# nickgreenquist/cu2rec

Measured on AMD Instinct MI355X. Metric: ratings/sec (SGD updates/sec), higher is better.
Workload: dtype f32

## Files before the change

cu2rec_amd/csrc/blocksolve.hip:

```cpp
#include <hip/hip_runtime.h>
#include <hip/hip_ext.h>

#include <algorithm>
#include <atomic>
#include <cmath>
#include <cstdlib>
#include <limits>
#include <mutex>
#include <string>
#include <utility>
#include <vector>

#include "blocksolve.hpp"
#include "blocksolve_device.hpp"
#include "blocksolve_gram.hpp"
#include "blocksolve_lookahead.hpp"
#include "blocksolve_solve.hpp"
#include "blocksolve_update.hpp"
#include "hip_check.hpp"

namespace cu2rec {

namespace {

using namespace bs_dev;

__global__ void bs_tables_kernel(SgdHyper h, float *__restrict__ t) {
    const int k = threadIdx.x;
    if (k > 2 * kB) return;
    const double a = 1.0 - static_cast<double>(h.lr) * static_cast<double>(h.q_reg);
    const double c = 1.0 - static_cast<double>(h.lr) * static_cast<double>(h.ib_reg);
    double ak = 1.0, ck = 1.0;
    for (int i = 0; i < k; ++i) {
        ak *= a;
        ck *= c;
    }
    t[kTabAdel + k] = static_cast<float>(1.0 - ak);
    t[kTabCdel + k] = static_cast<float>(1.0 - ck);
    t[kTabApow + k] = static_cast<float>(ak);
    t[kTabCpow + k] = static_cast<float>(ck);
}

__device__ __forceinline__ int lower_bound_key(const uint32_t *__restrict__ keys, int n, uint32_t target) {
    int lo = 0, hi = n;
    while (lo < hi) {
        const int mid = (lo + hi) >> 1;
        if (keys[mid] < target) lo = mid + 1; else hi = mid;
    }
    return lo;
}

__global__ __launch_bounds__(256) void bs_plan_kernel(const uint32_t *__restrict__ keys, int n_active, int n_hot,
                                                      int item_bits, int max_blocks, const int *__restrict__ item_of_rank,
                                                      int *__restrict__ chain_begin, BsChainDesc *__restrict__ chains,
                                                      BsBlockDesc *__restrict__ blocks, int *__restrict__ walk_begin, size_t stride) {
    __shared__ int s_part[256];
    const int b = blockIdx.x, tid = threadIdx.x;
    const uint32_t *kb = keys + static_cast<size_t>(b) * stride;
    int *cb = chain_begin + static_cast<size_t>(b) * (n_hot + 1);
    BsChainDesc *cd = chains + static_cast<size_t>(b) * max(n_hot, 1);
    BsBlockDesc *bd = blocks + static_cast<size_t>(b) * max_blocks;
    for (int r = tid; r <= n_hot; r += 256) cb[r] = lower_bound_key(kb, n_active, static_cast<uint32_t>(r));
    __syncthreads();
    if (tid == 0) walk_begin[b] = cb[n_hot];
    const int per = (n_hot + 255) / 256;
    const int r0 = min(tid * per, n_hot), r1 = min(r0 + per, n_hot);
    int mine = 0;
    for (int r = r0; r < r1; ++r) mine += (cb[r + 1] - cb[r] + kB - 1) / kB;
    s_part[tid] = mine;
    __syncthreads();
    __shared__ int s_total;
    if (tid == 0) {
        int run = 0;
        for (int t = 0; t < 256; ++t) {
            const int v = s_part[t];
            s_part[t] = run;
            run += v;
        }
        s_total = run;
    }
    __syncthreads();
    int off = s_part[tid];
    for (int r = r0; r < r1; ++r) {
        const int begin = cb[r], len = cb[r + 1] - begin;
        cd[r] = BsChainDesc{begin, len, off, item_of_rank[r]};
        const int nb = (len + kB - 1) / kB;
        for (int m = 0; m < nb; ++m) bd[off + m] = BsBlockDesc{begin + kB * m, min(kB, len - kB * m), r, m};
        off += nb;
    }
    for (int g = s_total + tid; g < max_blocks; g += 256) bd[g] = BsBlockDesc{0, 0, 0, 0};
}

__global__ __launch_bounds__(256, 4) void bs_gram_kernel(SgdArgs a, BsIteration it) {
    extern __shared__ float4 bs_smem[];
    const int g = static_cast<int>(blockIdx.x) - it.la_grid;
    __builtin_amdgcn_s_setprio(2);
    struct Through {
        unsigned long long *count;
        __device__ ~Through() {
            if (count && threadIdx.x == 0)
                __hip_atomic_fetch_add(count + 16 * (blockIdx.x & 31), 1ull, __ATOMIC_RELAXED, __HIP_MEMORY_SCOPE_AGENT);
        }
    } through_count{it.gram_done};
    if (g < 0) {
        const BsChainDesc last = it.chains[it.la_ranks - 1];
        const int la_end = min(last.blk0 + (last.len + kB - 1) / kB, it.la_cap);
        for (int gb = g + it.la_grid; gb < la_end; gb += it.la_grid) gram_cross_block(a, it, gb, bs_smem);
        return;
    }
    gram_block(a, it, g, bs_smem);
}

template <int SW>
__global__ __launch_bounds__(512) void bs_solve_kernel(SgdArgs a, BsIteration it) {
    extern __shared__ float4 bs_smem[];
    if (it.gram_done && threadIdx.x == 0)
        __hip_atomic_fetch_add(it.solve_started, 1ull, __ATOMIC_RELAXED, __HIP_MEMORY_SCOPE_AGENT);
    const int chain = blockIdx.x;
    const BsChainDesc cd = it.chains[chain];
    if constexpr (SW <= 8) {
        if (chain_is_lookahead(it, chain, cd)) {
            chain_lookahead<(4 * SW < kLaMaxSlots ? 4 * SW : kLaMaxSlots)>(a, it, bs_smem, cd);
            return;
        }
    }
    solve_chain<SW>(a, it, bs_smem, cd);
}

__global__ __launch_bounds__(64 * kUpdMaxWaves) void bs_update_kernel(SgdArgs a, BsIteration it) {
    const int g = blockIdx.x;
    __builtin_amdgcn_s_setprio(2);
    if (g == it.launch_blocks) {
        if (threadIdx.x == 0) await_iteration_end(it);
        return;
    }
    for (int blk = g; blk < it.max_blocks; blk += it.launch_blocks) {
        if (it.blocks[blk].n_valid == 0) break;
        update_block(a, it, blk);
    }
}

template <int SW>
void launch_solve_sw(const SgdArgs &a, const BsIteration &it, hipStream_t stream) {
    size_t lds = solve_lds_bytes(a.nslots, SW);
    if (it.la_ranks > 0) lds = std::max(lds, la_lds_bytes(a.nslots));
    ensure_max_dynamic_lds(reinterpret_cast<const void *>(bs_solve_kernel<SW>));
    hipLaunchKernelGGL((bs_solve_kernel<SW>), dim3(it.n_hot), dim3(512), lds, stream, a, it);
    const hipError_t err = hipGetLastError();
    if (err != hipSuccess)
        fail(CU2REC_EHIP, std::string("bs_solve_kernel launch failed: ") + hipGetErrorString(err) + " (SW " + std::to_string(SW) +
                              ", chains " + std::to_string(it.n_hot) + ", LDS " + std::to_string(lds) + " bytes)");
}

}

namespace {
__global__ void bs_probe_wait_kernel(const unsigned *word, unsigned *result, unsigned long long ticks) {
    if (threadIdx.x != 0) return;
    const unsigned long long t0 = wall_clock64();
    unsigned seen = 0;
    for (;;) {
        if (ld_agent(word) != 0u) {
            seen = 1;
            break;
        }
        __builtin_amdgcn_s_sleep(8);
        if (wall_clock64() - t0 > ticks) break;
    }
    __hip_atomic_store(result, seen ? 1u : 2u, __ATOMIC_RELAXED, __HIP_MEMORY_SCOPE_AGENT);
}

__global__ void bs_probe_signal_kernel(unsigned *word) {
    if (threadIdx.x == 0) __hip_atomic_store(word, 1u, __ATOMIC_RELAXED, __HIP_MEMORY_SCOPE_AGENT);
}

bool probe_streams(hipStream_t waiter, hipStream_t signaller, unsigned *scratch) {
    CU2REC_HIP(hipMemsetAsync(scratch, 0, 64 * sizeof(unsigned), waiter));
    CU2REC_HIP(hipStreamSynchronize(waiter));
    CU2REC_HIP(hipStreamSynchronize(signaller));
    hipLaunchKernelGGL(bs_probe_wait_kernel, dim3(1), dim3(64), 0, waiter, scratch, scratch + 32, 1000000ull);
    hipLaunchKernelGGL(bs_probe_signal_kernel, dim3(1), dim3(64), 0, signaller, scratch);
    CU2REC_HIP(hipGetLastError());
    CU2REC_HIP(hipStreamSynchronize(waiter));
    CU2REC_HIP(hipStreamSynchronize(signaller));
    unsigned result = 0;
    CU2REC_HIP(hipMemcpy(&result, scratch + 32, sizeof(unsigned), hipMemcpyDeviceToHost));
    return result == 1u;
}

int topology(DeviceRuntime &r, hipStream_t stream, hipStream_t side) {
    if (r.topology >= 0) return r.topology;
    if (const char *env = std::getenv("CU2REC_BS_GATE")) {
        r.topology = std::atoi(env) != 0 ? DeviceRuntime::kTopologyDevice : DeviceRuntime::kTopologyEvents;
        r.topology_forced = true;
        r.topology_why = std::string("CU2REC_BS_GATE=") + env;
        return r.topology;
    }
    if (const char *pmc = std::getenv("ROCPROF_COUNTER_COLLECTION"))
        if (*pmc && std::string(pmc) != "0" && std::string(pmc) != "False" && std::string(pmc) != "false") {
            r.topology = DeviceRuntime::kTopologyEvents;
            r.topology_why = "a rocprofv3 counter pass (ROCPROF_COUNTER_COLLECTION) serialises kernels across streams";
            return r.topology;
        }
    const bool forward = probe_streams(stream, side, r.probe);
    const bool backward = forward && probe_streams(side, stream, r.probe);
    if (forward && backward) {
        r.topology = DeviceRuntime::kTopologyDevice;
        r.topology_why = "two-stream handshake probe passed in both directions";
    } else {
        r.topology = DeviceRuntime::kTopologyEvents;
        r.topology_why = std::string("two-stream handshake probe: a wait kernel on the ") + (forward ? "side" : "main") +
                         " stream was not reached by the other stream's signal kernel within 10 ms (the streams do not run side by side here)";
    }
    return r.topology;
}

unsigned long long wait_ticks() {
    static const unsigned long long ticks = [] {
        double sec = 2.0;
        if (const char *env = std::getenv("CU2REC_BS_WAIT_S")) sec = std::max(0.001, std::atof(env));
        return static_cast<unsigned long long>(sec * 1e8);
    }();
    return ticks;
}

#ifdef CU2REC_TEST_HOOKS
int dbg() {
    static const int bits = std::getenv("CU2REC_BS_DBG") ? std::atoi(std::getenv("CU2REC_BS_DBG")) : 0;
    return bits;
}
#else
constexpr int dbg() { return 0; }
#endif

__global__ void bs_gate_kernel(const unsigned long long *count, unsigned long long target, const unsigned long long *started,
                               unsigned long long started_target, unsigned long long wait_ticks) {
    const int lane = threadIdx.x;
    const unsigned long long t0 = wall_clock64();
    unsigned polls = 0;
    for (;;) {
        unsigned long long v = lane < 32 ? ld_agent(count + 16 * lane) : 0ull;
#pragma unroll
        for (int off = 16; off > 0; off >>= 1) v += __shfl_xor(v, off);
        const unsigned long long sum = __shfl(v, 0);
        const unsigned long long st = ld_agent(started);
        if (sum >= target && st >= started_target) break;
        __builtin_amdgcn_s_sleep(16);
        if ((++polls & 63u) == 0 && wall_clock64() - t0 > wait_ticks) break;
    }
}

__global__ void bs_signal_kernel(unsigned long long *word, unsigned long long value) {
    if (threadIdx.x == 0) __hip_atomic_store(word, value, __ATOMIC_RELAXED, __HIP_MEMORY_SCOPE_AGENT);
}

void launch_gram(const SgdArgs &a, const BsIteration &it, hipStream_t stream, hipEvent_t stop) {
    const size_t gram_lds = gram_lds_bytes(a.nslots, it.la_ranks > 0);
    ensure_max_dynamic_lds(reinterpret_cast<const void *>(bs_gram_kernel));
    const int grid = it.max_blocks + (it.la_ranks > 0 ? it.la_grid : 0);
    if (stop) hipExtLaunchKernelGGL(bs_gram_kernel, dim3(grid), dim3(256), static_cast<uint32_t>(gram_lds), stream, nullptr, stop, 0, a, it);
    else hipLaunchKernelGGL(bs_gram_kernel, dim3(grid), dim3(256), gram_lds, stream, a, it);
    CU2REC_HIP(hipGetLastError());
}

void launch_solve(const SgdArgs &a, const BsIteration &it, hipStream_t stream) {
    const int sw = (a.nslots + 3) / 4;
    if (sw <= 1) launch_solve_sw<1>(a, it, stream);
    else if (sw <= 2) launch_solve_sw<2>(a, it, stream);
    else if (sw <= 4) launch_solve_sw<4>(a, it, stream);
    else if (sw <= 7) launch_solve_sw<7>(a, it, stream);
    else if (sw <= 8) launch_solve_sw<8>(a, it, stream);
    else if (sw <= 12) launch_solve_sw<12>(a, it, stream);
    else if (sw <= 16) launch_solve_sw<16>(a, it, stream);
    else fail(CU2REC_EUNSUPPORTED, "block-solve mode is compiled for n_factors <= 252");
}

void launch_update(const SgdArgs &a, const BsIteration &it, hipStream_t stream) {
    const int nwaves = (4 * a.nslots + 63) / 64;
    hipLaunchKernelGGL(bs_update_kernel, dim3(it.launch_blocks + (it.side_seq ? 1 : 0)), dim3(64 * nwaves), 0, stream, a, it);
    CU2REC_HIP(hipGetLastError());
}

std::atomic<int> g_lookahead{-1};
std::atomic<float> g_min_rate{-2.f};
constexpr float kDefaultRate = 240.f;

float min_rate_state() {
    float cur = g_min_rate.load();
    if (cur == -2.f) {
        float init = -1.f;
        if (const char *env = std::getenv("CU2REC_BLOCKSOLVE_RATE")) init = std::max(0.01f, static_cast<float>(std::atof(env)));
        g_min_rate.compare_exchange_strong(cur, init);
        cur = g_min_rate.load();
    }
    return cur;
}
}

int blocksolve_lookahead_blocks(int blocks) {
    int prev = g_lookahead.load();
    if (prev < 0) {
        const char *env = std::getenv("CU2REC_BLOCKSOLVE_LOOKAHEAD");
        const int init = env ? std::max(0, std::atoi(env)) : 24;
        g_lookahead.compare_exchange_strong(prev, init);
        prev = g_lookahead.load();
    }
    if (blocks >= 0) g_lookahead.store(blocks);
    return prev;
}

float blocksolve_min_rate(float rate) {
    const float prev = min_rate_state();
    if (rate > 0.f) g_min_rate.store(rate);
    else if (rate < 0.f) g_min_rate.store(-1.f);
    return prev > 0.f ? prev : -1.f;
}

int blocksolve_hot_items(const std::vector<double> &rate, int n_active, int rank_limit) {
    const float state = min_rate_state();
    float min_rate = state > 0.f ? state : kDefaultRate;
    const int n_cols = static_cast<int>(rate.size());
    if (state <= 0.f) {
        min_rate = std::max(30.f, min_rate * static_cast<float>(n_active) / 131072.f);
        if (n_cols > 0 && n_active <= 131072 / 4 && rate[0] < 350.0) min_rate = rate[0] >= 150.0 ? 60.f : std::numeric_limits<float>::infinity();
    }
    int n = 0;
    while (n < n_cols && rate[n] >= min_rate) ++n;
    return std::min(n, rank_limit);
}

BlockSolve::BlockSolve(int n_hot_, const std::vector<double> &rate, double hot_rate, int n_active_, int item_bits_, int max_batch_,
                       const int *item_of_rank_)
    : n_hot(n_hot_), n_active(n_active_), item_bits(item_bits_), max_batch(max_batch_), item_of_rank(item_of_rank_) {
    max_blocks = n_active / kBsLinks + n_hot + 1;
    const double bound = (hot_rate + 8.0 * std::sqrt(hot_rate) + 64.0) / kBsLinks + n_hot + 1;
    launch_blocks = std::max(1, bound >= static_cast<double>(max_blocks) ? max_blocks : static_cast<int>(bound));
    if (dbg() & 512) launch_blocks = std::min(3, max_blocks);
    const int la_min = blocksolve_lookahead_blocks(-1);
    double la_blocks = 0.0;
    while (la_min > 0 && la_ranks < n_hot && rate[la_ranks] >= static_cast<double>(la_min) * kBsLinks) {
        la_blocks += std::ceil(rate[la_ranks] / kBsLinks) + 1.0;
        ++la_ranks;
    }
    if (la_ranks > 0) la_cap = std::min(max_blocks, static_cast<int>(la_blocks * 1.25) + 4 * la_ranks + 8);
    for (int slot = 0; slot < 2; ++slot) {
        chain_begin[slot].allocate(static_cast<size_t>(max_batch) * (n_hot + 1));
        walk_begin[slot].allocate(max_batch);
        chains[slot].allocate(static_cast<size_t>(max_batch) * n_hot);
        blocks[slot].allocate(static_cast<size_t>(max_batch) * max_blocks);
    }
    tables.allocate(kBsTableFloats);
    Mbuf.allocate(static_cast<size_t>(max_blocks) * kBsRecFloats);
    ebuf.allocate(static_cast<size_t>(max_blocks) * kBsLinks);
    solve_started.allocate(16);
    solve_started.zero();
    gram_done.allocate(32 * 16);
    gram_done.zero();
    side_seq.allocate(16);
    side_seq.zero();
    if (la_cap > 0) Nbuf.allocate(static_cast<size_t>(la_cap) * kBsCrossFloats);
}

BlockSolve::~BlockSolve() {
    if (upd) (void)hipStreamDestroy(upd);
    for (hipEvent_t e : {ev_call, ev_upd, ev_gram})
        if (e) (void)hipEventDestroy(e);
}

void BlockSolve::plan(int slot, const uint32_t *sk, int nb, size_t stride, hipStream_t sched) {
    hipLaunchKernelGGL(bs_plan_kernel, dim3(nb), dim3(256), 0, sched, sk, n_active, n_hot, item_bits, max_blocks, item_of_rank,
                       chain_begin[slot].ptr, chains[slot].ptr, blocks[slot].ptr, walk_begin[slot].ptr, stride);
}

void BlockSolve::begin(const SgdArgs &a, hipStream_t stream) {
    if (a.nslots < 1 || a.nslots > kBsMaxSlots) fail(CU2REC_EUNSUPPORTED, "block-solve mode is compiled for n_factors <= 252");
    const bool same = tables_valid && tables_for.lr == a.h.lr && tables_for.q_reg == a.h.q_reg && tables_for.ib_reg == a.h.ib_reg;
    if (!same) {
        hipLaunchKernelGGL(bs_tables_kernel, dim3(1), dim3(192), 0, stream, a.h, tables.ptr);
        tables_for = a.h;
        tables_valid = true;
    }
    if (qstart_ld != a.ldq) {
        CU2REC_HIP(hipStreamSynchronize(stream));
        qstart.allocate(static_cast<size_t>(max_blocks) * a.ldq);
        qstart_ld = a.ldq;
    }
    if (!upd) {
        CU2REC_HIP(hipStreamCreateWithFlags(&upd, hipStreamNonBlocking));
        for (hipEvent_t *e : {&ev_call, &ev_upd, &ev_gram}) CU2REC_HIP(hipEventCreateWithFlags(e, hipEventDisableTiming));
    }
    unsigned *status = nullptr;
    {
        std::lock_guard<std::mutex> lock(device_runtime_mutex());
        DeviceRuntime &r = device_runtime();
        device_join = topology(r, stream, upd) == DeviceRuntime::kTopologyDevice;
        status = r.status + DeviceRuntime::kBlocksolveWord;
        host_status = r.host_status + 1;
    }
    CU2REC_HIP(hipEventRecord(ev_call, stream));
    CU2REC_HIP(hipStreamWaitEvent(upd, ev_call, 0));
    const bool la_on = la_ranks > 0 && la_supported(a.nslots);
    it = BsIteration{};
    it.n_active = n_active;
    it.n_hot = n_hot;
    it.item_mask = (1u << item_bits) - 1u;
    it.item_of_rank = item_of_rank;
    it.tables = tables.ptr;
    it.log2a = static_cast<float>(std::log2(1.0 - static_cast<double>(a.h.lr) * static_cast<double>(a.h.q_reg)));
    it.log2c = static_cast<float>(std::log2(1.0 - static_cast<double>(a.h.lr) * static_cast<double>(a.h.ib_reg)));
    it.Mbuf = Mbuf.ptr;
    it.ebuf = ebuf.ptr;
    it.qstart = qstart.ptr;
    it.max_blocks = max_blocks;
    it.launch_blocks = launch_blocks;
    it.la_ranks = la_on ? la_ranks : 0;
    it.la_cap = la_cap;
    it.la_grid = la_on ? la_cap : 0;
    it.Nbuf = Nbuf.ptr;
    it.status = status;
    it.solve_started = solve_started.ptr;
    it.wait_ticks = wait_ticks();
    if (device_join) {
        it.gram_done = gram_done.ptr;
        it.side_seq = side_seq.ptr;
    }
    upd_pending = false;
}

void BlockSolve::iteration(const SgdArgs &a, int slot, int b, const uint32_t *keys, const uint64_t *vals, bool last, hipStream_t stream,
                           const SideChains &side) {
    it.keys = keys;
    it.vals = vals;
    it.chains = chains[slot].ptr + static_cast<size_t>(b) * n_hot;
    it.blocks = blocks[slot].ptr + static_cast<size_t>(b) * max_blocks;
    it.walk_begin = walk_begin[slot].ptr + b;
    it.side_target = device_join ? side_seq_host + 1 : 0;
    if (upd_pending) CU2REC_HIP(hipStreamWaitEvent(stream, ev_upd, 0));
    launch_gram(a, it, stream, device_join ? nullptr : ev_gram);
    if (device_join) gram_done_target += static_cast<unsigned long long>(max_blocks + it.la_grid);
    else CU2REC_HIP(hipStreamWaitEvent(upd, ev_gram, 0));
    launch_solve(a, it, stream);
    if (device_join) {
        started_total += static_cast<unsigned long long>(n_hot);
        hipLaunchKernelGGL(bs_gate_kernel, dim3(1), dim3(64), 0, upd, gram_done.ptr, gram_done_target + ((dbg() & 32) ? (1ull << 40) : 0ull),
                           solve_started.ptr, started_total, it.wait_ticks);
        CU2REC_HIP(hipGetLastError());
    }
    side(upd, !device_join || last ? ev_upd : nullptr);
    if (device_join) {
        ++side_seq_host;
        if (!(dbg() & 16)) {
            hipLaunchKernelGGL(bs_signal_kernel, dim3(1), dim3(64), 0, upd, side_seq.ptr, side_seq_host);
            CU2REC_HIP(hipGetLastError());
        }
    }
    launch_update(a, it, stream);
    upd_pending = !device_join;
}

void BlockSolve::join(hipStream_t stream) {
    CU2REC_HIP(hipStreamWaitEvent(stream, ev_upd, 0));
    upd_pending = false;
}

void BlockSolve::end(hipStream_t stream) {
    CU2REC_HIP(hipMemcpyAsync(host_status, it.status, sizeof(unsigned), hipMemcpyDeviceToHost, stream));
}

}
```

cu2rec_amd/csrc/blocksolve.hpp:

```cpp
#pragma once

#include <functional>
#include <vector>

#include <hip/hip_runtime.h>

#include <cstddef>
#include <cstdint>

#include "hip_check.hpp"
#include "kernels.hpp"

namespace cu2rec {

constexpr int kBsLinks = 64;
constexpr int kBsTableStride = 2 * kBsLinks + 1;
constexpr int kBsTableFloats = 4 * kBsTableStride;
constexpr int kBsFactorFloats = 3 * 32 * 32;
constexpr int kBsRecFloats = kBsFactorFloats + kBsLinks;
constexpr int kBsCrossFloats = kBsLinks * kBsLinks;
constexpr int kBsMaxSlots = 63;

struct BsBlockDesc {
    int pos0;
    int n_valid;
    int chain;
    int m;
};

struct BsChainDesc {
    int begin, len;
    int blk0;
    int item;
};

struct BsIteration {
    const uint32_t *keys;
    const uint64_t *vals;
    int n_active;
    int n_hot;
    uint32_t item_mask;
    const BsChainDesc *chains;
    const BsBlockDesc *blocks;
    const int *walk_begin;
    const int *item_of_rank;
    const float *tables;
    float log2a, log2c;
    float *Mbuf;
    float *ebuf;
    float *qstart;
    int max_blocks;
    int launch_blocks;
    int la_ranks;
    int la_cap;
    int la_grid;
    float *Nbuf;
    unsigned *status;
    unsigned long long *solve_started;
    const unsigned long long *side_seq;
    unsigned long long side_target;
    unsigned long long *gram_done;
    unsigned long long wait_ticks;
};

float blocksolve_min_rate(float rate);
int blocksolve_lookahead_blocks(int blocks);
int blocksolve_hot_items(const std::vector<double> &rate, int n_active, int rank_limit);

class BlockSolve {
public:
    BlockSolve(int n_hot, const std::vector<double> &rate, double hot_rate, int n_active, int item_bits, int max_batch,
               const int *item_of_rank);
    ~BlockSolve();
    BlockSolve(const BlockSolve &) = delete;
    BlockSolve &operator=(const BlockSolve &) = delete;
    void plan(int slot, const uint32_t *sk, int nb, size_t stride, hipStream_t sched);
    void begin(const SgdArgs &a, hipStream_t stream);
    using SideChains = std::function<void(hipStream_t side, hipEvent_t stop)>;
    void iteration(const SgdArgs &a, int slot, int b, const uint32_t *keys, const uint64_t *vals, bool last, hipStream_t stream,
                   const SideChains &side);
    void join(hipStream_t stream);
    void end(hipStream_t stream);

    const int n_hot;

private:
    int n_active, item_bits, max_batch;
    const int *item_of_rank;
    int max_blocks;
    int launch_blocks;
    int la_ranks = 0;
    int la_cap = 0;
    DeviceBuffer<int> chain_begin[2], walk_begin[2];
    DeviceBuffer<BsChainDesc> chains[2];
    DeviceBuffer<BsBlockDesc> blocks[2];
    DeviceBuffer<float> tables, Mbuf, ebuf, qstart, Nbuf;
    int qstart_ld = 0;
    SgdHyper tables_for{};
    bool tables_valid = false;
    DeviceBuffer<unsigned long long> solve_started, gram_done, side_seq;
    unsigned long long gram_done_target = 0, started_total = 0, side_seq_host = 0;
    hipStream_t upd = nullptr;
    hipEvent_t ev_call = nullptr, ev_upd = nullptr, ev_gram = nullptr;
    BsIteration it{};
    bool device_join = false;
    bool upd_pending = false;
    unsigned *host_status = nullptr;
};

}
```

cu2rec_amd/csrc/ordered.hip:

```cpp
#include <hip/hip_runtime.h>
#include <hip/hip_ext.h>

#include <cstring>
#include <rocprim/rocprim.hpp>

#include <algorithm>
#include <atomic>
#include <cmath>
#include <cstdio>
#include <cstdlib>
#include <limits>
#include <map>
#include <mutex>
#include <numeric>
#include <string>
#include <vector>

#include "hip_check.hpp"
#include "item_rates.hpp"
#include "kernels.hpp"
#include "ordered.hpp"
#include "sampler.hpp"
#include "sgd_device.hpp"

namespace cu2rec {

namespace {

using namespace dev;

constexpr unsigned kSegBlock = 1024;
constexpr unsigned kSegItems = 8;
using SegSortConfig = rocprim::segmented_radix_sort_config<8, rocprim::kernel_config<kSegBlock, kSegItems>,
                                                           rocprim::WarpSortConfig<8, 4, 256, 64, 16, 8, 256>, true>;

constexpr int kHotChains = 256;

__device__ __forceinline__ int lower_bound_key(const uint32_t *__restrict__ keys, int n, uint32_t target) {
    int lo = 0, hi = n;
    while (lo < hi) {
        const int mid = (lo + hi) >> 1;
        if (keys[mid] < target) lo = mid + 1; else hi = mid;
    }
    return lo;
}

constexpr int kRowRounds = 8;
constexpr int kTileStride = 65;

__global__ __launch_bounds__(256) void schedule_keys_tile_kernel(const int *__restrict__ indptr, const int *__restrict__ indices,
                                                                 const float *__restrict__ data, const int *__restrict__ item_rank,
                                                                 int n_rows, int n_batch, int item_bits, uint32_t sentinel, uint64_t seed,
                                                                 uint64_t iter0, int user_offset, uint32_t *__restrict__ keys,
                                                                 uint64_t *__restrict__ vals) {
    __shared__ uint32_t t_key[64 * kTileStride];
    __shared__ uint32_t t_rat[64 * kTileStride];
    const int wave = threadIdx.x >> 6, lane = threadIdx.x & 63;
    const int x0 = static_cast<int>(blockIdx.x) * 64;
    const int b = lane;
    const int xi = min(x0 + 16 * wave + min(lane, 16), n_rows);
    const int bound = indptr[xi];
    for (int u0 = 0; u0 < 16; u0 += 4) {
        int low[4], high[4], y_i[4], y[4], vi[4][4];
        uint32_t r[4], vr[4][4];
        bool live[4];
#pragma unroll
        for (int j = 0; j < 4; ++j) {
            const int x = x0 + 16 * wave + u0 + j;
            low[j] = __shfl(bound, u0 + j);
            high[j] = __shfl(bound, u0 + j + 1);
            live[j] = x < n_rows && low[j] != high[j];
            const int last = max(high[j] - 1, low[j]);
#pragma unroll
            for (int k = 0; k < 4; ++k) {
                const int e = live[j] ? min(low[j] + 64 * k + lane, last) : 0;
                vi[j][k] = indices[e];
                vr[j][k] = __float_as_uint(data[e]);
            }
        }
#pragma unroll
        for (int j = 0; j < 4; ++j) {
            const int x = x0 + 16 * wave + u0 + j;
            y_i[j] = live[j] && b < n_batch ? sampler_index(seed, static_cast<uint64_t>(user_offset + x), iter0 + b, low[j], high[j]) : low[j];
            y[j] = 0;
            r[j] = 0;
        }
#pragma unroll
        for (int j = 0; j < 4; ++j) {
            if (!live[j]) continue;
            if (high[j] - low[j] <= 256 * kRowRounds) {
                for (int base = low[j]; base < high[j]; base += 256) {
                    if (base > low[j]) {
#pragma unroll
                        for (int k = 0; k < 4; ++k) {
                            const int e = min(base + 64 * k + lane, high[j] - 1);
                            vi[j][k] = indices[e];
                            vr[j][k] = __float_as_uint(data[e]);
                        }
                    }
                    const int pos = y_i[j] - base, src = pos & 63, kk = pos >> 6;
#pragma unroll
                    for (int k = 0; k < 4; ++k) {
                        const int yi = __shfl(vi[j][k], src);
                        const uint32_t ri = __shfl(vr[j][k], src);
                        if (kk == k && pos >= 0) y[j] = yi, r[j] = ri;
                    }
                }
            } else {
                y[j] = indices[y_i[j]];
                r[j] = __float_as_uint(data[y_i[j]]);
            }
        }
        int rank[4];
#pragma unroll
        for (int j = 0; j < 4; ++j) rank[j] = item_rank[y[j]];
#pragma unroll
        for (int j = 0; j < 4; ++j) {
            const uint32_t key = live[j] ? static_cast<uint32_t>(rank[j]) : sentinel;
            t_key[b * kTileStride + 16 * wave + u0 + j] = key;
            t_rat[b * kTileStride + 16 * wave + u0 + j] = live[j] ? r[j] : 0u;
        }
    }
    __syncthreads();
    const int x = x0 + lane;
    if (x < n_rows) {
        for (int bb = wave; bb < n_batch; bb += 4) {
            const uint32_t key = t_key[bb * kTileStride + lane];
            const size_t idx = static_cast<size_t>(bb) * n_rows + x;
            keys[idx] = key;
            vals[idx] = (key & sentinel) ? 0ull : (static_cast<uint64_t>(static_cast<uint32_t>(x)) << 32) | t_rat[bb * kTileStride + lane];
        }
    }
}

__global__ __launch_bounds__(kBlock) void chain_ranges_kernel(const uint32_t *__restrict__ keys, int n_active, int n_ranks,
                                                              int *__restrict__ ranges, size_t stride) {
    const int b = blockIdx.x;
    const uint32_t *kb = keys + static_cast<size_t>(b) * stride;
    for (int r = threadIdx.x; r <= n_ranks; r += kBlock)
        ranges[static_cast<size_t>(b) * (n_ranks + 1) + r] = lower_bound_key(kb, n_active, static_cast<uint32_t>(r));
}

template <int J>
__device__ __forceinline__ float chain_step(const SgdArgs &a, Row<J> &p, Row<J> &q, float ub, float &ib, float rating) {
    const float err = rating - predict<J>(p, q, ub, ib, a.global_bias);
    rank1_update<J>(p, q, err, a.h);
    ib = ib + a.h.lr * (err - a.h.ib_reg * ib);
    return ub + a.h.lr * (err - a.h.ub_reg * ub);
}

constexpr int kWide = 32;

typedef unsigned int uint2_t __attribute__((ext_vector_type(2)));

__device__ __forceinline__ float cross_row_sum(float v) {
    const uint2_t r = __builtin_amdgcn_permlane16_swap(__float_as_uint(v), __float_as_uint(v), false, false);
    return __uint_as_float(r.x) + __uint_as_float(r.y);
}

template <int W, int S>
struct DuoShape {
    static_assert(W == kGroup || S == 1, "the 32-lane layout holds exactly one slot per lane");
    static constexpr int kTile = S == 1 ? 8 : 4;
    static constexpr int kPart = kTile / 2;
    static constexpr int kChains = W == kWide ? 2 : (S <= 3 ? 4 : (S <= 6 ? 2 : 1));
};

template <int S>
struct WideRow {
    float4 v[S];
};

template <int W, int S>
struct DuoLds {
    static constexpr int T = DuoShape<W, S>::kTile;
    float4 p[2][T][S][W];
    float4 qold[2][T][S][W];
    float rating[2][T], ub[2][T], err[2][T];
    int user[2][T];
};

template <int W, int S>
struct DuoTileRegs {
    WideRow<S> rows[DuoShape<W, S>::kPart];
    uint64_t val;
    float ub;
};

template <int W, int S>
__device__ __forceinline__ WideRow<S> load_wide_row(const float *__restrict__ base, size_t row, int ld, int nslots, int lane) {
    const float4 *p = reinterpret_cast<const float4 *>(base + row * static_cast<size_t>(ld));
    WideRow<S> r;
#pragma unroll
    for (int s = 0; s < S; ++s) {
        const int slot = lane + W * s;
        const float4 v = p[min(slot, nslots - 1)];
        const bool ok = slot < nslots;
        r.v[s] = make_float4(ok ? v.x : 0.f, ok ? v.y : 0.f, ok ? v.z : 0.f, ok ? v.w : 0.f);
    }
    return r;
}

template <int W, int S>
__device__ __forceinline__ void store_wide_row(float *__restrict__ base, size_t row, int ld, int nslots, int lane,
                                               const WideRow<S> &r) {
    float4 *p = reinterpret_cast<float4 *>(base + row * static_cast<size_t>(ld));
#pragma unroll
    for (int s = 0; s < S; ++s) {
        const int slot = lane + W * s;
        if (slot < nslots) p[slot] = r.v[s];
    }
}

template <int W, int S>
__device__ __forceinline__ uint64_t duo_load_vals(const uint64_t *__restrict__ vals, int tile_start, int end, int part,
                                                  int lane) {
    constexpr int kPart = DuoShape<W, S>::kPart;
    return vals[min(tile_start + kPart * part + (lane & (kPart - 1)), end - 1)];
}

template <int W, int S>
__device__ __forceinline__ void duo_load_rows(DuoTileRegs<W, S> &r, const SgdArgs &a, uint64_t val, int lane) {
    r.val = val;
    const int my_user = static_cast<int>(val >> 32);
    r.ub = a.user_bias[my_user];
#pragma unroll
    for (int t = 0; t < DuoShape<W, S>::kPart; ++t) {
        const int x = __shfl(my_user, t, W);
        r.rows[t] = load_wide_row<W, S>(a.P, static_cast<size_t>(x), a.ldp, a.nslots, lane);
    }
}

template <int W, int S>
__device__ __forceinline__ void duo_publish(DuoLds<W, S> &l, int buf, const DuoTileRegs<W, S> &r, int part, int lane) {
    constexpr int kPart = DuoShape<W, S>::kPart;
#pragma unroll
    for (int t = 0; t < kPart; ++t)
#pragma unroll
        for (int s = 0; s < S; ++s) l.p[buf][kPart * part + t][s][lane] = r.rows[t].v[s];
    if (lane < kPart) {
        const int e = kPart * part + lane;
        l.rating[buf][e] = __uint_as_float(static_cast<uint32_t>(r.val));
        l.ub[buf][e] = r.ub;
        l.user[buf][e] = static_cast<int>(r.val >> 32);
    }
}

template <int W, int S>
__device__ __forceinline__ void duo_update_users(DuoLds<W, S> &l, int buf, int n_valid, const SgdArgs &a, int part, int lane) {
    constexpr int kPart = DuoShape<W, S>::kPart;
#pragma unroll
    for (int t = 0; t < kPart; ++t) {
        const int e = kPart * part + t;
        if (e < n_valid) {
            const float err = l.err[buf][e];
            WideRow<S> pn;
#pragma unroll
            for (int s = 0; s < S; ++s) {
                const float4 po = l.p[buf][e][s][lane], qo = l.qold[buf][e][s][lane];
                pn.v[s].x = step(po.x, qo.x, err, a.h.lr, a.h.p_reg);
                pn.v[s].y = step(po.y, qo.y, err, a.h.lr, a.h.p_reg);
                pn.v[s].z = step(po.z, qo.z, err, a.h.lr, a.h.p_reg);
                pn.v[s].w = step(po.w, qo.w, err, a.h.lr, a.h.p_reg);
            }
            store_wide_row<W, S>(a.P, static_cast<size_t>(l.user[buf][e]), a.ldp, a.nslots, lane, pn);
        }
    }
    const int mine = kPart * part + lane;
    if (lane < kPart && mine < n_valid) {
        const float ub = l.ub[buf][mine], err = l.err[buf][mine];
        a.user_bias[l.user[buf][mine]] = ub + a.h.lr * (err - a.h.ub_reg * ub);
    }
}

template <int W, int S>
__device__ __forceinline__ void duo_step_a(DuoLds<W, S> &l, int buf, int t, const WideRow<S> &po, float rating, float ub,
                                           const SgdArgs &a, WideRow<S> &q, float &ib, int lane) {
    float acc = slot_dot(q.v[0], po.v[0]);
#pragma unroll
    for (int s = 1; s < S; ++s) acc = acc + slot_dot(q.v[s], po.v[s]);
    const float dot = W == kWide ? row_sum16(cross_row_sum(acc)) : row_sum16(acc);
    const float err = rating - (((a.global_bias + ub) + ib) + dot);
#pragma unroll
    for (int s = 0; s < S; ++s) l.qold[buf][t][s][lane] = q.v[s];
    if (lane == 0) l.err[buf][t] = err;
#pragma unroll
    for (int s = 0; s < S; ++s) {
        const float4 qo = q.v[s];
        q.v[s].x = step(qo.x, po.v[s].x, err, a.h.lr, a.h.q_reg);
        q.v[s].y = step(qo.y, po.v[s].y, err, a.h.lr, a.h.q_reg);
        q.v[s].z = step(qo.z, po.v[s].z, err, a.h.lr, a.h.q_reg);
        q.v[s].w = step(qo.w, po.v[s].w, err, a.h.lr, a.h.q_reg);
    }
// ... 218 lines not shown
        walk_group<J>(a, keys, vals, n_active, item_of_rank, item_mask, n_hot, p);
}

template <int J>
void launch_chain(const SgdArgs &a, const uint32_t *keys, const uint64_t *vals, int n_active, const int *item_of_rank,
                  uint32_t item_mask, int n_hot, hipStream_t stream, int rank_lo, const int *ranges, hipEvent_t stop, int walk_bound) {
    const int chains_per_block = DuoShape<(J == 2 ? kWide : kGroup), (J == 2 ? 1 : J)>::kChains;
    const int hot_blocks = (std::max(n_hot - rank_lo, 0) + chains_per_block - 1) / chains_per_block;
    int walk_lo = 0;
    if (ranges && walk_bound < n_active) walk_lo = ((n_active - walk_bound) / kGroupsPerBlock) * kGroupsPerBlock;
    const int walk_blocks = (n_active - walk_lo + kGroupsPerBlock - 1) / kGroupsPerBlock;
    const int blocks = hot_blocks + walk_blocks + (walk_lo > 0 ? 1 : 0);
    if (blocks == 0) return;
    if (stop)
        hipExtLaunchKernelGGL(sgd_ordered_kernel<J>, dim3(blocks), dim3(kBlock), 0, stream, nullptr, stop, 0, a, keys, vals, n_active,
                              item_of_rank, item_mask, n_hot, hot_blocks, rank_lo, ranges, walk_lo, walk_blocks);
    else
        hipLaunchKernelGGL(sgd_ordered_kernel<J>, dim3(blocks), dim3(kBlock), 0, stream, a, keys, vals, n_active,
                           item_of_rank, item_mask, n_hot, hot_blocks, rank_lo, ranges, walk_lo, walk_blocks);
}

void launch_chains(const SgdArgs &a, const uint32_t *kb, const uint64_t *vb, int n_active, const int *item_of_rank,
                   uint32_t item_mask, int n_hot, hipStream_t stream, int rank_lo, const int *ranges, hipEvent_t stop, int walk_bound) {
    dispatch_row_width(a.nslots, [&](auto j) {
        launch_chain<j()>(a, kb, vb, n_active, item_of_rank, item_mask, n_hot, stream, rank_lo, ranges, stop, walk_bound);
    });
}

int bits_for(int n) {
    int b = 1;
    while ((1ll << b) < n) ++b;
    return b;
}

}

OrderedSchedule::OrderedSchedule(const int *d_indptr, const int *d_indices, int n_rows_, int n_cols_, int nnz_)
    : n_rows(n_rows_), n_cols(n_cols_), nnz(nnz_) {
    require(d_indptr && n_rows >= 0 && n_cols > 0 && nnz >= 0, "ordered schedule: bad argument");
    require_device();
    std::vector<int> indptr(static_cast<size_t>(n_rows) + 1), indices(static_cast<size_t>(std::max(nnz, 1)));
    CU2REC_HIP(hipMemcpy(indptr.data(), d_indptr, indptr.size() * sizeof(int), hipMemcpyDeviceToHost));
    if (nnz) CU2REC_HIP(hipMemcpy(indices.data(), d_indices, static_cast<size_t>(nnz) * sizeof(int), hipMemcpyDeviceToHost));
    n_active = 0;
    for (int u = 0; u < n_rows; ++u) n_active += indptr[u + 1] > indptr[u];
    std::vector<double> rate(n_cols);
    std::vector<int> order(n_cols), rank(n_cols);
    for (int u = 0; u < n_rows; ++u) require(indptr[u] <= indptr[u + 1] && indptr[u + 1] <= nnz, "ordered schedule: bad indptr");
    item_update_rates(indptr.data(), indices.data(), n_rows, n_cols, rate.data());
    std::iota(order.begin(), order.end(), 0);
    std::stable_sort(order.begin(), order.end(), [&](int l, int r) { return rate[l] > rate[r]; });
    for (int r = 0; r < n_cols; ++r) rank[order[r]] = r;
    item_rank.allocate(n_cols);
    item_rank.upload(rank.data(), n_cols);
    item_of_rank.allocate(n_cols);
    item_of_rank.upload(order.data(), n_cols);
    std::vector<double> rank_rate(n_cols);
    for (int r = 0; r < n_cols; ++r) rank_rate[r] = rate[order[r]];
    rank_rate_prefix.assign(static_cast<size_t>(n_cols) + 1, 0.0);
    for (int r = 0; r < n_cols; ++r) rank_rate_prefix[r + 1] = rank_rate_prefix[r] + rank_rate[r];
    item_bits = bits_for(n_cols);
    int b_bits = std::min(6, 31 - item_bits - 1);
    require(b_bits >= 0, "ordered schedule: too many items for 32-bit keys");
    max_batch = 1 << b_bits;
    while (max_batch > 1 && static_cast<size_t>(max_batch) * n_rows > (size_t(1) << 27)) max_batch >>= 1;
    const size_t cap = static_cast<size_t>(max_batch) * std::max(n_rows, 1);
    for (int slot = 0; slot < 2; ++slot)
        for (int i = 0; i < 2; ++i) {
            keys[slot][i].allocate(cap);
            vals[slot][i].allocate(cap);
        }
    temp_bytes = 0;
    {
        std::vector<int> offs(static_cast<size_t>(max_batch) + 1);
        for (int b = 0; b <= max_batch; ++b) offs[b] = static_cast<int>(static_cast<size_t>(b) * n_rows);
        seg_offsets.allocate(offs.size());
        seg_offsets.upload(offs.data(), offs.size());
        CU2REC_HIP(rocprim::segmented_radix_sort_pairs<SegSortConfig>(nullptr, temp_bytes, keys[0][0].ptr, keys[0][1].ptr, vals[0][0].ptr,
                                                                       vals[0][1].ptr, static_cast<unsigned>(cap), static_cast<unsigned>(max_batch),
                                                                       seg_offsets.ptr, seg_offsets.ptr + 1, 0u, 32u, nullptr));
    }
    temp.allocate(temp_bytes + 16);
    const int n_hot_bs = blocksolve_hot_items(rank_rate, n_active, (1 << item_bits) - 1);
    if (n_hot_bs > 0)
        bs.reset(new BlockSolve(n_hot_bs, rank_rate, rank_rate_prefix[static_cast<size_t>(n_hot_bs)], n_active, item_bits, max_batch,
                                item_of_rank.ptr));
    n_duo_bs = n_hot_bs;
    while (n_duo_bs < n_cols && n_duo_bs < 4096 && rank_rate[n_duo_bs] >= 12.0) ++n_duo_bs;
    n_duo_bs = std::min(n_duo_bs, (1 << item_bits) - 1);
    n_range_ranks = std::max(std::max(std::min(n_cols, kHotChains), n_duo_bs), n_hot_bs);
    n_range_ranks = std::min(n_range_ranks, (1 << item_bits) - 1);
    for (int slot = 0; slot < 2; ++slot) chain_ranges[slot].allocate(static_cast<size_t>(max_batch) * (n_range_ranks + 1));
    {
        int lo = 0, hi = 0;
        CU2REC_HIP(hipDeviceGetStreamPriorityRange(&lo, &hi));
        CU2REC_HIP(hipStreamCreateWithPriority(&sched, hipStreamNonBlocking, lo));
    }
    for (int slot = 0; slot < 2; ++slot) {
        CU2REC_HIP(hipEventCreateWithFlags(&ev_ready[slot], hipEventDisableTiming));
        CU2REC_HIP(hipEventCreateWithFlags(&ev_consumed[slot], hipEventDisableTiming));
    }
    CU2REC_HIP(hipEventCreateWithFlags(&ev_last, hipEventDisableTiming));
}

OrderedSchedule::~OrderedSchedule() {
    if (have_last) (void)hipEventSynchronize(ev_last);
    if (sched) (void)hipStreamSynchronize(sched);
    if (sched) (void)hipStreamDestroy(sched);
    for (int slot = 0; slot < 2; ++slot) {
        if (ev_ready[slot]) (void)hipEventDestroy(ev_ready[slot]);
        if (ev_consumed[slot]) (void)hipEventDestroy(ev_consumed[slot]);
    }
    if (ev_last) (void)hipEventDestroy(ev_last);
}

int OrderedSchedule::walk_bound(int n_hot) const {
#ifdef CU2REC_TEST_HOOKS
    if (const char *env = std::getenv("CU2REC_BS_DBG"))
        if (std::atoi(env) & 256) return 16;
#endif
    const int r = std::min(std::max(n_hot, 0), n_cols);
    const double mean = std::max(0.0, static_cast<double>(n_active) - rank_rate_prefix[static_cast<size_t>(r)]);
    const double bound = mean + 8.0 * std::sqrt(mean) + 64.0;
    return bound >= static_cast<double>(n_active) ? n_active : static_cast<int>(bound);
}

void OrderedSchedule::run(SgdArgs a, uint64_t iter0, int n_iters, hipStream_t stream, bool blocksolve) {
    if (n_active == 0) return;
    if (blocksolve && !bs) blocksolve = false;
    if (blocksolve && (1.0 - static_cast<double>(a.h.lr) * static_cast<double>(a.h.q_reg) <= 0.0 ||
                       1.0 - static_cast<double>(a.h.lr) * static_cast<double>(a.h.ib_reg) <= 0.0))
        blocksolve = false;
    if (have_last && last_stream != stream) CU2REC_HIP(hipStreamWaitEvent(stream, ev_last, 0));
    if (blocksolve) bs->begin(a, stream);
    const uint32_t item_mask = (1u << item_bits) - 1u;
    const int n_hot = std::min(std::min(n_cols, kHotChains), static_cast<int>(item_mask));
    const int n_hot_bs = blocksolve_items(), n_side = std::max(n_duo_bs, n_hot_bs);
    const int walk_bound_plain = walk_bound(n_hot), walk_bound_bs = walk_bound(n_side);
    const size_t seg = static_cast<size_t>(n_rows);
    auto schedule = [&](int slot, uint64_t first_iter, int nb) {
        win[slot].valid = false;
        const size_t n = static_cast<size_t>(nb) * n_rows;
        if (slot_used[slot]) CU2REC_HIP(hipStreamWaitEvent(sched, ev_consumed[slot], 0));
        hipLaunchKernelGGL(schedule_keys_tile_kernel, dim3((n_rows + 63) / 64), dim3(256), 0, sched, a.indptr, a.indices, a.data,
                           item_rank.ptr, n_rows, nb, item_bits, 1u << item_bits, a.seed, first_iter, a.user_offset, keys[slot][0].ptr,
                           vals[slot][0].ptr);
        CU2REC_HIP(hipGetLastError());
        size_t bytes = temp_bytes;
        CU2REC_HIP(rocprim::segmented_radix_sort_pairs<SegSortConfig>(temp.ptr, bytes, keys[slot][0].ptr, keys[slot][1].ptr, vals[slot][0].ptr,
                                                                       vals[slot][1].ptr, static_cast<unsigned>(n), static_cast<unsigned>(nb),
                                                                       seg_offsets.ptr, seg_offsets.ptr + 1, 0u,
                                                                       static_cast<unsigned>(item_bits + 1), sched));
        Window w{true, a.seed, first_iter, nb, a.user_offset, a.indptr, blocksolve, keys[slot][1].ptr, vals[slot][1].ptr};
        hipLaunchKernelGGL(chain_ranges_kernel, dim3(nb), dim3(kBlock), 0, sched, w.sk, n_active, n_range_ranks, chain_ranges[slot].ptr, seg);
        CU2REC_HIP(hipGetLastError());
        if (blocksolve) bs->plan(slot, w.sk, nb, seg, sched);
        CU2REC_HIP(hipEventRecord(ev_ready[slot], sched));
        slot_used[slot] = true;
        win[slot] = w;
    };
    struct DropWindows {
        OrderedSchedule *s;
        ~DropWindows() {
            if (!s->speculate) s->win[0].valid = s->win[1].valid = false;
        }
    } drop_windows{this};
    auto holds = [&](const Window &w, uint64_t it) {
        return w.valid && w.seed == a.seed && w.user_offset == a.user_offset && w.indptr == a.indptr && w.blocksolve == blocksolve &&
               it >= w.iter_begin && it < w.iter_begin + static_cast<uint64_t>(w.nb);
    };
    const uint32_t *kb = nullptr;
    const uint64_t *vb = nullptr;
    const int *ranges = nullptr;
    const BlockSolve::SideChains side_chains = [&](hipStream_t side, hipEvent_t stop) {
        launch_chains(a, kb, vb, n_active, item_of_rank.ptr, item_mask, n_side, side, n_hot_bs, ranges, stop, walk_bound_bs);
    };
    int done = 0;
    while (done < n_iters) {
        const uint64_t it_first = iter0 + static_cast<uint64_t>(done);
        int slot = holds(win[0], it_first) ? 0 : (holds(win[1], it_first) ? 1 : -1);
        if (slot < 0) {
            CU2REC_HIP(hipEventRecord(ev_consumed[1], stream));
            CU2REC_HIP(hipStreamWaitEvent(sched, ev_consumed[1], 0));
            slot_used[1] = true;
            win[1].valid = false;
            schedule(0, it_first, std::min(max_batch, n_iters - done));
            slot = 0;
        }
        const int off = static_cast<int>(it_first - win[slot].iter_begin);
        const int nb = std::min(n_iters - done, win[slot].nb - off);
        const uint64_t next_begin = win[slot].iter_begin + static_cast<uint64_t>(win[slot].nb);
        const long long call_beyond = static_cast<long long>(iter0 + static_cast<uint64_t>(n_iters)) - static_cast<long long>(next_begin);
        const int next_nb = speculate ? max_batch : static_cast<int>(std::min<long long>(max_batch, call_beyond));
        bool next_scheduled = (holds(win[slot ^ 1], next_begin) && win[slot ^ 1].iter_begin == next_begin) || next_nb <= 0;
        auto schedule_next = [&] {
            if (next_scheduled) return;
            next_scheduled = true;
            schedule(slot ^ 1, next_begin, next_nb);
        };
        CU2REC_HIP(hipStreamWaitEvent(stream, ev_ready[slot], 0));
        const uint32_t *sk = win[slot].sk + static_cast<size_t>(off) * seg;
        const uint64_t *sv = win[slot].sv + static_cast<size_t>(off) * seg;
        a.iters = 1;
        for (int b = 0; b < nb; ++b) {
            if (b == std::min(2, nb - 1) && b > 0) schedule_next();
            a.iter0 = iter0 + done + b;
            kb = sk + static_cast<size_t>(b) * seg;
            vb = sv + static_cast<size_t>(b) * seg;
            ranges = chain_ranges[slot].ptr + static_cast<size_t>(off + b) * (n_range_ranks + 1);
            if (blocksolve) bs->iteration(a, slot, off + b, kb, vb, b == nb - 1, stream, side_chains);
            else
                launch_chains(a, kb, vb, n_active, item_of_rank.ptr, item_mask, n_hot, stream, 0, n_hot <= n_range_ranks ? ranges : nullptr,
                              nullptr, walk_bound_plain);
        }
        schedule_next();
        CU2REC_HIP(hipGetLastError());
        if (blocksolve) bs->join(stream);
        CU2REC_HIP(hipEventRecord(ev_consumed[slot], stream));
        done += nb;
    }
    if (blocksolve) bs->end(stream);
    CU2REC_HIP(hipEventRecord(ev_last, stream));
    last_stream = stream;
    have_last = true;
}

}
```

cu2rec_amd/csrc/sampler.hpp:

```cpp
#pragma once

#include <cstdint>

#if defined(__HIPCC__)
#include <hip/hip_runtime.h>
#define CU2REC_HD __host__ __device__ __forceinline__
#else
#define CU2REC_HD inline
#endif

namespace cu2rec {

CU2REC_HD uint32_t mulhi32(uint32_t a, uint32_t b) {
#if defined(__HIP_DEVICE_COMPILE__)
    return __umulhi(a, b);
#else
    return static_cast<uint32_t>((static_cast<uint64_t>(a) * b) >> 32);
#endif
}

CU2REC_HD uint32_t philox4x32_10_word0(uint32_t c0, uint32_t c1, uint32_t c2, uint32_t c3, uint32_t k0, uint32_t k1) {
    constexpr uint32_t M0 = 0xD2511F53u, M1 = 0xCD9E8D57u, W0 = 0x9E3779B9u, W1 = 0xBB67AE85u;
#pragma unroll
    for (int round = 0; round < 9; ++round) {
        const uint32_t hi0 = mulhi32(M0, c0), lo0 = M0 * c0;
        const uint32_t hi1 = mulhi32(M1, c2), lo1 = M1 * c2;
        c0 = hi1 ^ c1 ^ k0;
        c1 = lo1;
        c2 = hi0 ^ c3 ^ k1;
        c3 = lo0;
        k0 += W0;
        k1 += W1;
    }
    return mulhi32(M1, c2) ^ c1 ^ k0;
}

CU2REC_HD uint32_t sampler_draw(uint64_t seed, uint64_t user, uint64_t iteration) {
    return philox4x32_10_word0(static_cast<uint32_t>(iteration), static_cast<uint32_t>(iteration >> 32),
                               static_cast<uint32_t>(user), static_cast<uint32_t>(user >> 32),
                               static_cast<uint32_t>(seed), static_cast<uint32_t>(seed >> 32));
}

CU2REC_HD float sampler_uniform(uint32_t x) {
    const float inv = 2.3283064365386963e-10f;
    return inv + static_cast<float>(x) * inv;
}

CU2REC_HD int sampler_index(uint64_t seed, uint64_t user, uint64_t iteration, int low, int high) {
    const float u = sampler_uniform(sampler_draw(seed, user, iteration));
#if defined(__HIP_DEVICE_COMPILE__)
    const float c = ceilf(u * static_cast<float>(high - low));
#else
    const float c = __builtin_ceilf(u * static_cast<float>(high - low));
#endif
    return static_cast<int>(c) - 1 + low;
}

}
```

Before: 1.780 billion.

## Build chain ranges by key scan, reuse them in block-solve plan, trim loads

The chain-range kernel stops running one binary search per rank. It scans the sorted keys once and writes each rank's start at the positions where the key value jumps, using 1024-thread blocks. The block-solve planner now reads these shared ranges instead of running its own binary searches and keeping a separate chain_begin buffer. Smaller edits are also included: readlane replaces shfl for uniform bounds, 64-wide pieces beyond a row's end are skipped in the tile kernel, and the Philox multiply is done as a single 64-bit product. The risk is that a scan over all active keys may cost more than the searches when n_active is much larger than the rank count.

```diff
diff --git a/cu2rec_amd/csrc/blocksolve.hip b/cu2rec_amd/csrc/blocksolve.hip
--- a/cu2rec_amd/csrc/blocksolve.hip
+++ b/cu2rec_amd/csrc/blocksolve.hip
@@ -41,27 +41,14 @@
     t[kTabCpow + k] = static_cast<float>(ck);
 }
 
-__device__ __forceinline__ int lower_bound_key(const uint32_t *__restrict__ keys, int n, uint32_t target) {
-    int lo = 0, hi = n;
-    while (lo < hi) {
-        const int mid = (lo + hi) >> 1;
-        if (keys[mid] < target) lo = mid + 1; else hi = mid;
-    }
-    return lo;
-}
-
-__global__ __launch_bounds__(256) void bs_plan_kernel(const uint32_t *__restrict__ keys, int n_active, int n_hot,
-                                                      int item_bits, int max_blocks, const int *__restrict__ item_of_rank,
-                                                      int *__restrict__ chain_begin, BsChainDesc *__restrict__ chains,
-                                                      BsBlockDesc *__restrict__ blocks, int *__restrict__ walk_begin, size_t stride) {
+__global__ __launch_bounds__(256) void bs_plan_kernel(const int *__restrict__ ranges, int range_stride, int n_hot, int max_blocks,
+                                                      const int *__restrict__ item_of_rank, BsChainDesc *__restrict__ chains,
+                                                      BsBlockDesc *__restrict__ blocks, int *__restrict__ walk_begin) {
     __shared__ int s_part[256];
     const int b = blockIdx.x, tid = threadIdx.x;
-    const uint32_t *kb = keys + static_cast<size_t>(b) * stride;
-    int *cb = chain_begin + static_cast<size_t>(b) * (n_hot + 1);
+    const int *cb = ranges + static_cast<size_t>(b) * range_stride;
     BsChainDesc *cd = chains + static_cast<size_t>(b) * max(n_hot, 1);
     BsBlockDesc *bd = blocks + static_cast<size_t>(b) * max_blocks;
-    for (int r = tid; r <= n_hot; r += 256) cb[r] = lower_bound_key(kb, n_active, static_cast<uint32_t>(r));
-    __syncthreads();
     if (tid == 0) walk_begin[b] = cb[n_hot];
     const int per = (n_hot + 255) / 256;
     const int r0 = min(tid * per, n_hot), r1 = min(r0 + per, n_hot);
@@ -344,7 +331,6 @@
     }
     if (la_ranks > 0) la_cap = std::min(max_blocks, static_cast<int>(la_blocks * 1.25) + 4 * la_ranks + 8);
     for (int slot = 0; slot < 2; ++slot) {
-        chain_begin[slot].allocate(static_cast<size_t>(max_batch) * (n_hot + 1));
         walk_begin[slot].allocate(max_batch);
         chains[slot].allocate(static_cast<size_t>(max_batch) * n_hot);
         blocks[slot].allocate(static_cast<size_t>(max_batch) * max_blocks);
@@ -367,9 +353,10 @@
         if (e) (void)hipEventDestroy(e);
 }
 
-void BlockSolve::plan(int slot, const uint32_t *sk, int nb, size_t stride, hipStream_t sched) {
-    hipLaunchKernelGGL(bs_plan_kernel, dim3(nb), dim3(256), 0, sched, sk, n_active, n_hot, item_bits, max_blocks, item_of_rank,
-                       chain_begin[slot].ptr, chains[slot].ptr, blocks[slot].ptr, walk_begin[slot].ptr, stride);
+void BlockSolve::plan(int slot, const int *ranges, int range_stride, int nb, hipStream_t sched) {
+    require(range_stride > n_hot, "block-solve plan: the chain ranges stop short of the hot chains");
+    hipLaunchKernelGGL(bs_plan_kernel, dim3(nb), dim3(256), 0, sched, ranges, range_stride, n_hot, max_blocks, item_of_rank, chains[slot].ptr,
+                       blocks[slot].ptr, walk_begin[slot].ptr);
 }
 
 void BlockSolve::begin(const SgdArgs &a, hipStream_t stream) {
diff --git a/cu2rec_amd/csrc/blocksolve.hpp b/cu2rec_amd/csrc/blocksolve.hpp
--- a/cu2rec_amd/csrc/blocksolve.hpp
+++ b/cu2rec_amd/csrc/blocksolve.hpp
@@ -74,7 +74,7 @@
     ~BlockSolve();
     BlockSolve(const BlockSolve &) = delete;
     BlockSolve &operator=(const BlockSolve &) = delete;
-    void plan(int slot, const uint32_t *sk, int nb, size_t stride, hipStream_t sched);
+    void plan(int slot, const int *ranges, int range_stride, int nb, hipStream_t sched);
     void begin(const SgdArgs &a, hipStream_t stream);
     using SideChains = std::function<void(hipStream_t side, hipEvent_t stop)>;
     void iteration(const SgdArgs &a, int slot, int b, const uint32_t *keys, const uint64_t *vals, bool last, hipStream_t stream,
@@ -91,7 +91,7 @@
     int launch_blocks;
     int la_ranks = 0;
     int la_cap = 0;
-    DeviceBuffer<int> chain_begin[2], walk_begin[2];
+    DeviceBuffer<int> walk_begin[2];
     DeviceBuffer<BsChainDesc> chains[2];
     DeviceBuffer<BsBlockDesc> blocks[2];
     DeviceBuffer<float> tables, Mbuf, ebuf, qstart, Nbuf;
diff --git a/cu2rec_amd/csrc/ordered.hip b/cu2rec_amd/csrc/ordered.hip
--- a/cu2rec_amd/csrc/ordered.hip
+++ b/cu2rec_amd/csrc/ordered.hip
@@ -47,6 +47,8 @@
 
 constexpr int kRowRounds = 8;
 constexpr int kTileStride = 65;
+
+__device__ __forceinline__ bool has_piece(int base, int k, int high) { return k == 0 || base + 64 * k < high; }
 
 __global__ __launch_bounds__(256) void schedule_keys_tile_kernel(const int *__restrict__ indptr, const int *__restrict__ indices,
                                                                  const float *__restrict__ data, const int *__restrict__ item_rank,
@@ -67,12 +69,13 @@
 #pragma unroll
         for (int j = 0; j < 4; ++j) {
             const int x = x0 + 16 * wave + u0 + j;
-            low[j] = __shfl(bound, u0 + j);
-            high[j] = __shfl(bound, u0 + j + 1);
+            low[j] = __builtin_amdgcn_readlane(bound, u0 + j);
+            high[j] = __builtin_amdgcn_readlane(bound, u0 + j + 1);
             live[j] = x < n_rows && low[j] != high[j];
             const int last = max(high[j] - 1, low[j]);
 #pragma unroll
             for (int k = 0; k < 4; ++k) {
+                if (!has_piece(low[j], k, high[j])) continue;
                 const int e = live[j] ? min(low[j] + 64 * k + lane, last) : 0;
                 vi[j][k] = indices[e];
                 vr[j][k] = __float_as_uint(data[e]);
@@ -93,6 +96,7 @@
                     if (base > low[j]) {
 #pragma unroll
                         for (int k = 0; k < 4; ++k) {
+                            if (!has_piece(base, k, high[j])) continue;
                             const int e = min(base + 64 * k + lane, high[j] - 1);
                             vi[j][k] = indices[e];
                             vr[j][k] = __float_as_uint(data[e]);
@@ -101,6 +105,7 @@
                     const int pos = y_i[j] - base, src = pos & 63, kk = pos >> 6;
 #pragma unroll
                     for (int k = 0; k < 4; ++k) {
+                        if (!has_piece(base, k, high[j])) continue;
                         const int yi = __shfl(vi[j][k], src);
                         const uint32_t ri = __shfl(vr[j][k], src);
                         if (kk == k && pos >= 0) y[j] = yi, r[j] = ri;
@@ -133,12 +138,32 @@
     }
 }
 
-__global__ __launch_bounds__(kBlock) void chain_ranges_kernel(const uint32_t *__restrict__ keys, int n_active, int n_ranks,
-                                                              int *__restrict__ ranges, size_t stride) {
+constexpr int kRangeBlock = 1024, kRangeUnroll = 8;
+
+__global__ __launch_bounds__(kRangeBlock) void chain_ranges_kernel(const uint32_t *__restrict__ keys, int n_active, int n_ranks,
+                                                                   int *__restrict__ ranges, size_t stride) {
     const int b = blockIdx.x;
     const uint32_t *kb = keys + static_cast<size_t>(b) * stride;
-    for (int r = threadIdx.x; r <= n_ranks; r += kBlock)
-        ranges[static_cast<size_t>(b) * (n_ranks + 1) + r] = lower_bound_key(kb, n_active, static_cast<uint32_t>(r));
+    int *rb = ranges + static_cast<size_t>(b) * (n_ranks + 1);
+    const uint32_t top = static_cast<uint32_t>(n_ranks);
+    for (int base = threadIdx.x; base <= n_active; base += kRangeBlock * kRangeUnroll) {
+        uint32_t key[kRangeUnroll], prev[kRangeUnroll];
+#pragma unroll
+        for (int k = 0; k < kRangeUnroll; ++k) {
+            const int p = base + k * kRangeBlock;
+            const uint32_t here = kb[min(p, n_active - 1)], before = kb[min(max(p - 1, 0), n_active - 1)];
+            key[k] = p < n_active ? here : ~0u;
+            prev[k] = before;
+        }
+#pragma unroll
+        for (int k = 0; k < kRangeUnroll; ++k) {
+            const int p = base + k * kRangeBlock;
+            if (p > n_active) break;
+            const uint32_t lo = p > 0 ? prev[k] + 1u : 0u, hi = min(key[k], top);
+            for (uint32_t r = lo; r <= hi; ++r) rb[r] = p;
+        }
+        if (key[kRangeUnroll - 1] >= top) break;
+    }
 }
 
 template <int J>
@@ -663,9 +688,9 @@
                                                                        seg_offsets.ptr, seg_offsets.ptr + 1, 0u,
                                                                        static_cast<unsigned>(item_bits + 1), sched));
         Window w{true, a.seed, first_iter, nb, a.user_offset, a.indptr, blocksolve, keys[slot][1].ptr, vals[slot][1].ptr};
-        hipLaunchKernelGGL(chain_ranges_kernel, dim3(nb), dim3(kBlock), 0, sched, w.sk, n_active, n_range_ranks, chain_ranges[slot].ptr, seg);
+        hipLaunchKernelGGL(chain_ranges_kernel, dim3(nb), dim3(kRangeBlock), 0, sched, w.sk, n_active, n_range_ranks, chain_ranges[slot].ptr, seg);
         CU2REC_HIP(hipGetLastError());
-        if (blocksolve) bs->plan(slot, w.sk, nb, seg, sched);
+        if (blocksolve) bs->plan(slot, chain_ranges[slot].ptr, n_range_ranks + 1, nb, sched);
         CU2REC_HIP(hipEventRecord(ev_ready[slot], sched));
         slot_used[slot] = true;
         win[slot] = w;
diff --git a/cu2rec_amd/csrc/sampler.hpp b/cu2rec_amd/csrc/sampler.hpp
--- a/cu2rec_amd/csrc/sampler.hpp
+++ b/cu2rec_amd/csrc/sampler.hpp
@@ -19,16 +19,24 @@
 #endif
 }
 
+struct PhiloxProduct {
+    uint32_t hi, lo;
+};
+
+CU2REC_HD PhiloxProduct mul32x32(uint32_t a, uint32_t b) {
+    const uint64_t p = static_cast<uint64_t>(a) * b;
+    return PhiloxProduct{static_cast<uint32_t>(p >> 32), static_cast<uint32_t>(p)};
+}
+
 CU2REC_HD uint32_t philox4x32_10_word0(uint32_t c0, uint32_t c1, uint32_t c2, uint32_t c3, uint32_t k0, uint32_t k1) {
     constexpr uint32_t M0 = 0xD2511F53u, M1 = 0xCD9E8D57u, W0 = 0x9E3779B9u, W1 = 0xBB67AE85u;
 #pragma unroll
     for (int round = 0; round < 9; ++round) {
-        const uint32_t hi0 = mulhi32(M0, c0), lo0 = M0 * c0;
-        const uint32_t hi1 = mulhi32(M1, c2), lo1 = M1 * c2;
-        c0 = hi1 ^ c1 ^ k0;
-        c1 = lo1;
-        c2 = hi0 ^ c3 ^ k1;
-        c3 = lo0;
+        const PhiloxProduct p0 = mul32x32(M0, c0), p1 = mul32x32(M1, c2);
+        c0 = p1.hi ^ c1 ^ k0;
+        c1 = p1.lo;
+        c2 = p0.hi ^ c3 ^ k1;
+        c3 = p0.lo;
         k0 += W0;
         k1 += W1;
     }
```

After: 1.751 billion. -1.7%, worse.
